# tbuckworth/train-procgen-pytorch

Hardware: AMD Instinct MI355X
Metric: env steps/sec (whole node), coinrun hard-500 IMPALA-CNN PPO (higher is better)
Workload: dtype bf16

## Files before the change

### train-procgen-pytorch_amd/csrc/common.h

```cpp
#pragma once
#include <hip/hip_runtime.h>
#include <stdint.h>
#include <stddef.h>

typedef float f32x4 __attribute__((ext_vector_type(4)));

#define MI_WAVE 64

#if defined(__HIPCC__)
typedef float mi_f32x2 __attribute__((ext_vector_type(2)));
typedef __bf16 mi_bf16x2 __attribute__((ext_vector_type(2)));
__device__ __forceinline__ unsigned mi_pk_bf16(float lo, float hi) {
    return __builtin_bit_cast(unsigned, __builtin_convertvector((mi_f32x2){lo, hi}, mi_bf16x2));
}

typedef short mi_s16x2 __attribute__((ext_vector_type(2)));
constexpr unsigned MI_KEY_MIN2 = 0x80008000u;
__device__ __forceinline__ unsigned mi_bf16x2_to_keys(unsigned w) {
    const mi_s16x2 v = __builtin_bit_cast(mi_s16x2, w), s = v >> (mi_s16x2){15, 15};
    return __builtin_bit_cast(unsigned, (mi_s16x2)((v ^ (s & (mi_s16x2){0x7fff, 0x7fff})) - s));
}
__device__ __forceinline__ unsigned mi_keys_to_bf16x2(unsigned kk) {
    mi_s16x2 k = __builtin_bit_cast(mi_s16x2, kk);
    const mi_s16x2 s = k >> (mi_s16x2){15, 15};
// ... 121 lines not shown
    int n, A;
    float inv_n_global;
    LossHP hp;
    int value_from_logits;
};
int  loss_blocks(int n);
void launch_loss_fwd(const LossArgs& a, hipStream_t st);
void launch_loss_finalize(const LossArgs& a, int nblk, int phase, const float* fs_ptr, float* log_slot, hipStream_t st);
void launch_logp_all(const float* hout, int n, int A, float* lp_out, float* value_out, hipStream_t st, int value_from_logits = 0);
void launch_loss_bwd(const LossArgs& a, hipStream_t st);
constexpr int MI_MAX_SEG = 16;
constexpr int FS_PARTS = 8;
struct SegTab { int n_seg; int start[MI_MAX_SEG + 1]; };
int  loss_blocks_seg(const SegTab& st);
void launch_loss_fwd_seg(const LossArgs& a, const SegTab& st, bool with_bwd, hipStream_t stream);
void launch_loss_finalize_seg(const LossArgs& a, const SegTab& st, int phase, float* stats_base, const double* fs_parts, int fs_d, float* fs_out,
                              float* log_base, hipStream_t stream);
void launch_loss_finalize_records(const LossArgs& a, int n_rec, float* stats_base, const float* fs_base, float* log_base, hipStream_t stream);
void launch_fs_metric_seg(const void* flat_pre, int bf16, const SegTab& st, int d, float* colmax_scratch, double* fs_parts, hipStream_t stream);
int  fs_groups_per_segment(int n_seg);
void launch_fs_grad(const void* x, int bf16, int n, int d, const float* part, int G, void* Gd, float fs_coef, float* colmax, int* arg, hipStream_t st);
void launch_fs_keys(const void* x, int bf16, int n, int d, const float* part, int G, const int32_t* gpos, float* colmax, int* arg,
                    long long* keys, long long* keys_local, hipStream_t st);
void launch_fs_apply_keys(void* Gd, int bf16, int d, const long long* keys, const long long* keys_local, const int* arg, float fs_coef, hipStream_t st);
void launch_fs_from_keys(const long long* keys, int d, float* fs_out, hipStream_t st);
int  fs_metric_groups();
void launch_fs_metric(const void* flat_pre, int bf16, int n, int d, float* colmax_scratch, float* fs_out, hipStream_t st);

void launch_gae(const float* rew, const float* done, const float* value, float* adv, float* ret, int T, int E,
                float gamma, float lmbda, int use_gae, hipStream_t st);
// ... 86 lines not shown
```

### train-procgen-pytorch_amd/csrc/engine.hip

```cpp
#include "engine_ctx.h"

thread_local std::string g_err;
thread_local hipStream_t tl_stream = nullptr;
thread_local float* tl_ws = nullptr;
thread_local size_t tl_ws_floats = 0;
const char* mi_last_error(void) { return g_err.c_str(); }

#define NCCLC(x)                                                                                         \
    do {                                                                                                 \
        ncclResult_t r_ = (x);                                                                           \
        if (r_ != ncclSuccess) return fail(-5, std::string(#x) + ": " + ncclGetErrorString(r_) + " @" + std::to_string(__LINE__)); \
    } while (0)

extern "C" int mi_comm_destroy(mi_ctx* c);
static void prof_harvest(mi_ctx* c);
static const char* kProfNames[PC_COUNT] = {
    "conv_fwd_3_16_64", "conv_fwd_16_16_32", "conv_fwd_16_32_32", "conv_fwd_32_32_16", "conv_fwd_32_32_8",
    "conv_dgrad_3_16_64(unused)", "conv_dgrad_16_16_32", "conv_dgrad_16_32_32", "conv_dgrad_32_32_16", "conv_dgrad_32_32_8",
    "conv_wgrad_3_16_64", "conv_wgrad_16_16_32", "conv_wgrad_16_32_32", "conv_wgrad_32_32_16", "conv_wgrad_32_32_8",
    "maxpool_fwd", "maxpool_bwd", "gemm", "slab_reduce",
    "resblock_fwd_(unused)", "resblock_fwd_16_16_32", "resblock_fwd_(unused)", "resblock_fwd_32_32_16", "resblock_fwd_32_32_8",
    "resblock_dgrad_(unused)", "resblock_dgrad_16_16_32", "resblock_dgrad_(unused)", "resblock_dgrad_32_32_16", "resblock_dgrad_32_32_8"};
struct GroupJob { int t; const void* frames; size_t bytes; bool pull; bool have_rd, last; const float* u; unsigned long long seed; unsigned ticket; };
struct GroupWorker {
// ... 137 lines not shown
            "impala out_dim (output_dim) must be a multiple of 64 in [64, 512]");
    int ndev = 0;
    if (hipGetDeviceCount(&ndev) != hipSuccess || ndev == 0) return fail(-3, "no HIP device: the MI355X library has no CPU fallback");
    HIPC(hipSetDevice(cfg->device));
    mi_ctx* c = new mi_ctx();
    c->cfg = *cfg;
    c->T = cfg->n_steps; c->E = cfg->n_envs; c->A = cfg->n_actions;
    c->H = (cfg->arch == MI_ARCH_IMPALA && cfg->out_dim == 0) ? 256 : cfg->out_dim;
    c->NB = cfg->max_batch < cfg->n_envs ? cfg->n_envs : cfg->max_batch;
    c->bf = (cfg->arch == MI_ARCH_IMPALA) && cfg->precision == 1;
    c->lse = cfg->value_from_logits;
    c->es = c->bf ? 2.0 : 4.0;
    if (cfg->stream) { c->stream = (hipStream_t)cfg->stream; c->own_stream = false; }
    else { HIPC(hipStreamCreateWithFlags(&c->stream, hipStreamNonBlocking)); c->own_stream = true; }
    HIPC(hipEventCreateWithFlags(&c->ev_side_fork, hipEventDisableTiming)); HIPC(hipEventCreateWithFlags(&c->ev_side_join, hipEventDisableTiming));
    c->side_stream = nullptr; c->side_on = true; c->side.armed = false;
    if (cfg->arch == MI_ARCH_IMPALA) build_impala_layout(c); else build_mlp_layout(c);
    if (cfg->arch == MI_ARCH_IMPALA && !impala_regions_ok(c)) { delete c; return fail(-1, "internal: parameter layout does not split at embedder.fc.weight"); }

    const int64_t P = c->n_params, T = c->T, E = c->E, NB = c->NB;
    HIPC(dalloc(&c->params, P)); HIPC(dalloc(&c->grads, P)); HIPC(dalloc(&c->adam_m, P)); HIPC(dalloc(&c->adam_v, P));
    HIPC(dalloc(&c->rew, T * E)); HIPC(dalloc(&c->done, T * E)); HIPC(dalloc(&c->logp, T * E));
    HIPC(dalloc(&c->adv, T * E)); HIPC(dalloc(&c->ret, T * E)); HIPC(dalloc(&c->value, (T + 1) * E));
    HIPC(dalloc(&c->act, T * E)); HIPC(dalloc(&c->adv_stats, 4));
    c->frames = nullptr; c->obsf = nullptr; c->stage_frames = nullptr; c->stage_obs = nullptr;
    if (cfg->arch == MI_ARCH_IMPALA) {
        c->obs_bytes_per_env = 64 * 64 * 3;
        HIPC(dalloc(&c->frames, (size_t)(T + 1) * E * c->obs_bytes_per_env));
        HIPC(dalloc(&c->stage_frames, (size_t)NB * c->obs_bytes_per_env));
        const int chan[4] = {3, 16, 32, 32};
        int hin = 64;
// ... 615 lines not shown
            conv_wgrad(c, L[0], c->blk[b - 1].P2, nullptr, 0, c->GC, n);
            conv_dgrad(c, L[0], c->GC, nullptr, nullptr, Gout, n);
        }
    }
    conv_wgrad_reduce_all(c, n);
    issue_grad_allreduce(c, 0, c->fc.w_off, true);
}

static void fork_stats_and_fc(mi_ctx* c, int n) {
    fc_refresh(c);
    const mi_ctx::SideJob& j = c->side;
    hipStream_t ss = side_stream(c);
    hipStreamWaitEvent(ss, c->ev_side_fork, 0);
    if (c->idx_ev_deferred >= 0) { hipEventRecord(c->idx_ev[c->idx_ev_deferred], ss); c->idx_ev_deferred = -1; }
    tl_stream = ss;
    launch_heads_bwd_reduce(c->gemm_ws, c->grads + c->wh_off, c->grads + c->bh_off, n, c->H, c->A + 1, ss);
    launch_fs_metric_seg(c->blk[2].P2, c->bf, j.st, 2048, c->fs_scratch, c->fs_parts, ss);
    launch_loss_finalize_seg(j.a, j.st, j.mode, j.ring, c->fs_parts, 2048, j.fsr, j.log, ss);
    launch_fc_tn(c->dfeat, (const unsigned short*)c->blk[2].P2, c->grads + c->fc.w_off, c->gemm_ws, (size_t)8 << 20, c->H, 2048, n, ss);
    launch_colsum_acc(c->dfeat, n, c->H, c->H, c->grads + c->fc.b_off, c->col_ws, ss);
    tl_stream = nullptr;
    hipEventRecord(c->ev_side_join, ss);
    c->side.armed = false;
}
static int fork_slab_sums(mi_ctx* c, bool fork_recorded) {
    hipStream_t ss = side_stream(c);
    int max_len = 0;
    for (int q = 0; q < c->slab_desc_n; ++q) max_len = std::max(max_len, c->h_slab_desc[q].slab_len);
    if (!fork_recorded) hipEventRecord(c->ev_side_fork, c->stream);
    hipStreamWaitEvent(ss, c->ev_side_fork, 0);
    launch_reduce_all_slabs(c->slabs, c->grads, c->d_slab_desc, c->slab_desc_n, max_len, ss);
// ... 76 lines not shown
        backward_conv_pool_bf16(c, b, n, Gout, Ga);
        std::swap(Gout, Ga);
    }
    const bool fork2_on_launch = backward_residual_pair(c, 0, n, Gout, Ga, Gb, fork2 ? c->ev_side_fork : nullptr);
    c->sal_src = Gout;
    int slabs_done = 0;
    if (fork2 && c->slab_desc_n >= 1) slabs_done = fork_slab_sums(c, fork2_on_launch);
    conv_wgrad(c, c->convs[0], nullptr, &src, 0, Gout, n, c->blk[0].PI);
    if (fork1 || slabs_done) hipStreamWaitEvent(c->stream, c->ev_side_join, 0);
    conv_wgrad_reduce_all(c, n, slabs_done);
    issue_grad_allreduce(c, 0, c->fc.w_off, true);
}

static void net_backward(mi_ctx* c, const InputSrc& src, int n) {
    const bool impala = c->cfg.arch == MI_ARCH_IMPALA;
    if (!c->bwd_from_dfeat) {
        const bool to_side = c->side.armed && !tl_stream;
        heads_backward(c, n, impala ? 1 : 0, c->H <= 256 && c->A + 1 <= 16 && !tl_ws, true, CUR(c), !to_side, to_side ? c->ev_side_fork : nullptr);
    }
    if (!impala) backward_mlp(c, n);
    else if (!c->bf) backward_impala_fp32(c, src, n);
    else backward_impala_bf16(c, src, n);
}

static int upload_u(mi_ctx* c, const float* u, hipStream_t st, int row0, int rows, const float** du) {
    *du = nullptr;
    if (u) { HIPC(hipMemcpyAsync(c->d_u + row0, u, (size_t)rows * 4, hipMemcpyHostToDevice, st)); *du = c->d_u + row0; }
    return 0;
}
static int read_back_staged(mi_ctx* c, const int32_t* d_act, const float* d_logp, const float* d_val, int64_t* act_out, float* logp_out, float* value_out, void* extra_out = nullptr, const void* d_extra = nullptr, size_t extra_bytes = 0) {
    const size_t E = c->E;
// ... 451 lines not shown
    a.value_from_logits = c->lse;
    a.hp = LossHP{hp->eps_clip, hp->value_coef, hp->entropy_coef, hp->x_entropy_coef, hp->entropy_multiplier, hp->fs_coef};
    return a;
}
static void loss_and_records(mi_ctx* c, const LossArgs& a, const SegTab& st, bool with_dY, int mode, float* ring, float* fsr, float* log) {
    const bool impala = c->cfg.arch == MI_ARCH_IMPALA;
    if (impala) launch_fs_metric_seg(c->blk[2].P2, c->bf, st, 2048, c->fs_scratch, c->fs_parts, c->stream);
    launch_loss_fwd_seg(a, st, with_dY, c->stream);
    launch_loss_finalize_seg(a, st, mode, ring, impala ? c->fs_parts : nullptr, 2048, fsr, log, c->stream);
}

static bool side_eligible(const mi_ctx* c, int n, bool batch_terms) {
    return c->side_on && c->cfg.arch == MI_ARCH_IMPALA && c->bf && n >= 1024 && !batch_terms && !c->ar_armed && !c->comm && !c->bwd_from_dfeat &&
           c->H <= 256 && c->A + 1 <= 16;
}
static int minibatch_impl(mi_ctx* c, const int64_t* idx, int32_t n, const int32_t* seg_n, int32_t n_seg, int32_t n_global, const mi_hparams* hp) {
    ARG(c && hp, "null"); JOIN(c); ARG(n >= 0 && n <= c->NB, "n_idx must be in [0, max_batch]"); ARG(n_global >= 1, "n_global");
    ARG(n == 0 || idx, "idx"); ARG(n_seg >= 1 && n_seg <= MI_MAX_SEG && seg_n, "1 .. 16 segments");
    ARG(c->log_count + n_seg <= c->log_cap, "loss log full: call mi_loss_log_read(reset=1)");
    ARG(c->pending_n < 0, "previous multirank minibatch not finished");
    { long long tot = 0; for (int k = 0; k < n_seg; ++k) { ARG(seg_n[k] >= 0, "negative segment"); tot += seg_n[k]; } ARG(tot == n, "segments do not add up to n_idx"); }
    const bool batch_terms = hp->x_entropy_coef != 0.f || hp->fs_coef != 0.f;
    ARG(hp->fs_coef == 0.f || c->multirank != 2, "fs_coef != 0 needs the column maxima over the GLOBAL minibatch before the backward pass: multirank mode 1");
    ARG(hp->fs_coef == 0.f || c->multirank == 0 || c->cfg.arch != MI_ARCH_IMPALA || c->gpos_n == n,
        "fs_coef != 0 on several ranks: call mi_minibatch_positions with this pass's global minibatch positions first");
    ARG(n_seg == 1 || (!batch_terms && c->multirank != 1), "several minibatches per call need x_entropy_coef == 0, fs_coef == 0 and multirank mode 0 or 2");
    const int64_t TE = (int64_t)c->T * c->E;
    for (int k = 0; k < n; ++k) ARG(idx[k] >= 0 && idx[k] < TE, "minibatch index out of range");
    if (n)
        if (int r = stage_indices(c, n, [&](int32_t* h) { for (int k = 0; k < n; ++k) h[k] = (int32_t)idx[k]; }, side_eligible(c, n, batch_terms) && c->multirank != 1)) return r;
    InputSrc src = minibatch_src(c);
    c->prof.phase = 1;
    c->prof.sample_now = (c->prof.mb_count++ % c->prof.period) == 0;
    c->rec_last = false;
    net_forward(c, src, n, {.train = true});
    const bool impala = c->cfg.arch == MI_ARCH_IMPALA;
    LossArgs a = loss_args(c, n, n_global, hp);
    if (c->multirank == 2)
        ARG(!batch_terms, "multirank mode 2 needs x_entropy_coef == 0 and fs_coef == 0 (use mode 1)");
    if (c->multirank != 1) {
        SegTab st{};
        st.n_seg = n_seg;
        for (int k = 0; k < n_seg; ++k) st.start[k + 1] = st.start[k] + seg_n[k];
        float* ring = c->stats_ring + (size_t)c->log_count * 32;
        float* fsr = c->fs_ring + c->log_count;
        a.stats = ring;
        const int mode = c->multirank == 2 ? 1 : 3;
        float* log = c->multirank == 2 ? nullptr : c->loss_log + (size_t)c->log_count * 8;
        if (side_eligible(c, n, batch_terms)) {
            launch_loss_fwd_seg(a, st, true, c->stream);
            c->side = mi_ctx::SideJob{true, a, st, mode, ring, fsr, log};
        } else
            loss_and_records(c, a, st, !batch_terms, mode, ring, fsr, log);
        c->ring_args = a;
        c->log_count += n_seg;
        if (batch_terms) launch_loss_bwd(a, c->stream);
        if (impala && hp->fs_coef != 0.f && n > 0) { c->fs_grad_coef = hp->fs_coef; c->fs_G = fs_groups_per_segment(n_seg); }
        net_backward(c, src, n);
        c->fs_grad_coef = 0.f;
        HIPC(hipGetLastError()); NETCHK(c);
        return 0;
    }
    if (impala) launch_fs_metric(c->blk[2].P2, c->bf, n, 2048, c->fs_scratch, c->fs_val, c->stream);
    c->fs_global_pending = impala && hp->fs_coef != 0.f;
    if (c->fs_global_pending) {
        if (n > 0) launch_fs_keys(c->blk[2].P2, c->bf, n, 2048, c->fs_scratch, fs_metric_groups(), c->d_gpos, c->fs_colmax, c->fs_arg, c->fs_keys, c->fs_keys_local, c->stream);
// ... 261 lines not shown
    return 0;
}

int mi_device_ptr(mi_ctx* c, int32_t which, void** ptr, int64_t* n) {
    ARG(c && ptr && n, "null"); JOIN(c);
    switch (which) {
        case MI_PTR_GRADS: *ptr = c->grads; *n = c->n_params; return 0;
        case MI_PTR_LOSS_STATS: *ptr = c->loss_stats; *n = 32; return 0;
        case MI_PTR_PARAMS: *ptr = c->params; *n = c->n_params; return 0;
        case MI_PTR_STATS_RING: *ptr = c->stats_ring; *n = (int64_t)c->log_cap * 32; return 0;
        case MI_PTR_FS_KEYS: ARG(c->fs_keys, "IMPALA contexts only"); *ptr = c->fs_keys; *n = 2048; return 0;
        default: return fail(-1, "unknown pointer id");
    }
}

int mi_debug_flags(mi_ctx* c, int32_t flags) { ARG(c, "null"); JOIN(c); c->rollout_tail = !(flags & 1); c->no_pull = (flags & 4) != 0; c->side_on = !(flags & 16); return 0; }
```

### train-procgen-pytorch_amd/csrc/engine_ctx.h

```cpp
#pragma once
#include "common.h"
#include "../../include/mi355ppo.h"
#include <rccl/rccl.h>
#include <math.h>
#include <stdio.h>
#include <string.h>
#include <string>
#include <unordered_map>
#include <vector>
#include <atomic>
#include <chrono>
#include <condition_variable>
#include <mutex>
#include <thread>

#pragma clang diagnostic ignored "-Wc++20-designator"
#define MI_INTERNAL __attribute__((visibility("hidden")))

MI_INTERNAL extern thread_local std::string g_err;
MI_INTERNAL extern thread_local hipStream_t tl_stream;
MI_INTERNAL extern thread_local float* tl_ws;
MI_INTERNAL extern thread_local size_t tl_ws_floats;
#define CUR(c) (tl_stream ? tl_stream : (c)->stream)
static inline int fail(int code, const std::string& msg) { g_err = msg; return code; }
// ... 84 lines not shown
    bool gru_on; float *gru_wih, *gru_whh, *gru_bih, *gru_bhh, *h_state, *h_masked, *gru_gi, *gru_gh, *d_done;
    float *gru_x, *gru_dg; bool sal_keep_x, bwd_from_dfeat;
    static constexpr int IDX_RING = 32;
    int32_t* h_idx_ring[IDX_RING]; hipEvent_t idx_ev[IDX_RING]; bool idx_used[IDX_RING]; int idx_next, idx_ev_deferred;
    float* h_f; int32_t* h_i; size_t h_f_floats;
    int multirank;
    LossArgs pending; int pending_n;
    static constexpr int MAX_GROUPS = 4;
    int n_groups; hipStream_t main_stream, gs[MAX_GROUPS]; hipEvent_t ev_fork[MAX_GROUPS], ev_join[MAX_GROUPS];
    bool g_forked[MAX_GROUPS], g_busy[MAX_GROUPS], g_last[MAX_GROUPS], g_dirty[MAX_GROUPS]; unsigned g_ticket[MAX_GROUPS]; bool groups_live;
    struct GroupWorker* gw[MAX_GROUPS];
    std::atomic<int64_t> copy_slot_ns{0}; double copy_rate_bytes_per_us;
    std::unordered_map<const void*, bool> pull_ok; bool no_pull;
    hipStream_t side_stream; hipEvent_t ev_side_fork, ev_side_join;
    bool side_on;
    struct SideJob { bool armed; LossArgs a; SegTab st; int mode; float* ring; float* fsr; float* log; } side;
    bool rollout_tail;
    float *fs_colmax, fs_grad_coef; int *fs_arg, fs_G;
    long long *fs_keys, *fs_keys_local; int32_t *d_gpos, *h_gpos; int gpos_n; bool fs_global_pending, fs_global_apply;
    ncclComm_t comm, comm_grad; int comm_world, comm_rank; hipStream_t comm_stream; hipEvent_t ev_ar_ready, ev_ar_done;
    bool ar_armed, ar_issued, ar_inflight; double* adv_all;
    std::string net_err; std::mutex net_err_mu;
    float *h_ring, *h_rec_stage; hipEvent_t ev_rec; bool g_rec_ok[MAX_GROUPS];
    bool gru_train, rec_last; float *gru_g, *gru_m, *gru_v; double* gru_sumsq;
    float *rec_x, *rec_gi, *rec_sv, *rec_dgi, *rec_dgh, *rec_hm, *rec_mask, *rec_h0;
};

static inline char* obs_ring(mi_ctx* c) { return c->frames ? (char*)c->frames : (char*)c->obsf; }

MI_INTERNAL std::string net_err_take(mi_ctx* c);
MI_INTERNAL void net_err_set(mi_ctx* c, const std::string& m);
// ... 19 lines not shown
```

### train-procgen-pytorch_amd/csrc/engine_ops.hip

```cpp
#include "engine_ctx.h"

static int shape_of(int cin, int cout, int hw, ConvShape* s) {
    for (int k = 0; k < CS_COUNT; ++k) {
        int a, b, h; conv_shape_dims((ConvShape)k, &a, &b, &h);
        if (a == cin && b == cout && h == hw) { *s = (ConvShape)k; return 0; }
    }
    return fail(-1, "unsupported conv shape");
}

std::vector<uint16_t> host_to_bf16(const float* x, size_t n) {
    std::vector<uint16_t> o(n);
    for (size_t k = 0; k < n; ++k) { uint32_t u; memcpy(&u, x + k, 4); o[k] = (uint16_t)((u + 0x7FFFu + ((u >> 16) & 1u)) >> 16); }
    return o;
}
static void host_from_bf16(const uint16_t* h, float* x, size_t n) {
    for (size_t k = 0; k < n; ++k) { const uint32_t u = ((uint32_t)h[k]) << 16; memcpy(x + k, &u, 4); }
}
struct OpMem {
    static constexpr size_t GUARD = 64 * 1024;
    static constexpr int CANARY = 0xA5;
    struct Band { std::string name; unsigned char* p; size_t bytes; bool rezero; };
    const char* hook; hipStream_t st;
    std::vector<void*> owned;
    std::vector<Band> bands;
// ... 369 lines not shown
    if (graph) hipGraphDestroy(graph);
    c->prof.on = prof_on;
    HIPC(hipGetLastError()); NETCHK(c);
    return 0;
}

int mi_debug_read(mi_ctx* c, int32_t which, int32_t n, float* out) {
    ARG(c && out, "null"); JOIN(c); ARG(n >= 1 && n <= c->NB, "n must be in [1, max_batch]");
    if (which == 100 || which == 101 || which == 102) {
        ARG(which == 100 || c->rec_last, "which = 101 / 102: only after mi_minibatch_rec");
        const float* srcp = which == 102 ? c->dfeat : (which == 100 && c->rec_last) ? c->rec_x : c->feat;
        HIPC(hipMemcpyAsync(out, srcp, (size_t)n * c->H * 4, hipMemcpyDeviceToHost, c->stream));
        HIPC(hipStreamSynchronize(c->stream));
        return 0;
    }
    ARG(c->cfg.arch == MI_ARCH_IMPALA && which >= 0 && which < 24 && (which & 7) <= 5, "which");
    const Block& k = c->blk[which >> 3];
    const size_t pe = (size_t)n * (k.hin / 2) * (k.hin / 2) * k.cout;
    HIPC(hipStreamSynchronize(c->stream));
    if ((which & 7) == 5) {
        std::vector<uint8_t> h(pe);
        HIPC(hipMemcpy(h.data(), k.PI, pe, hipMemcpyDeviceToHost));
        for (size_t i = 0; i < pe; ++i) out[i] = (float)h[i];
        return 0;
    }
    const float* src[5] = {k.P0, k.A1, k.P1, k.A2, k.P2};
    return download_act(c, src[which & 7], out, pe);
}

int mi_op_maxpool(mi_ctx* c, int32_t mode, int32_t n, int32_t hw, int32_t ch, const float* in, const float* dout, float* out) {
// ... 63 lines not shown
```

### train-procgen-pytorch_amd/csrc/misc.hip

```cpp
#include "common.h"
#include <hip/hip_ext.h>
#include <math.h>
#include <stdlib.h>

static thread_local const char* tl_launch_err = nullptr;
void mi_launch_fail(const char* msg) { if (!tl_launch_err) tl_launch_err = msg; }
const char* mi_launch_failed_take() { const char* m = tl_launch_err; tl_launch_err = nullptr; return m; }

#define MFMA16(a, b, c) __builtin_amdgcn_mfma_f32_16x16x4f32((a), (b), (c), 0, 0, 0)

template <typename T>
__device__ __forceinline__ T wave_sum(T v) {
#pragma unroll
    for (int o = 32; o > 0; o >>= 1) v += __shfl_down(v, o, 64);
    return v;
}
__device__ __forceinline__ float wave_max(float v) {
#pragma unroll
    for (int o = 32; o > 0; o >>= 1) v = fmaxf(v, __shfl_down(v, o, 64));
    return v;
}
template <typename T>
__device__ __forceinline__ T block_sum256(T v, T* sbuf) {
    v = wave_sum(v);
// ... 380 lines not shown
            for (int q = 0; q < 8; ++q) v[q] = dY[(long long)(m + q * groups) * ld + n];
#pragma unroll
            for (int q = 0; q < 8; ++q) s += v[q];
        }
        for (; m < M; m += groups) s += dY[(long long)m * ld + n];
        part[(long long)rg * N + n] = s;
    }
}
void launch_colsum_acc(const float* dY, int M, int N, int ld, float* db, float* col_ws, hipStream_t st) {
    if (M <= 0) return;
    const int gy = (M >= 4096 && N <= 1024) ? 64 : 16;
    hipLaunchKernelGGL(colsum_partial_kernel, dim3((N + 63) / 64, gy), dim3(256), 0, st, dY, M, N, ld, col_ws);
    launch_reduce_slabs(col_ws, gy * 4, N, db, N, nullptr, 0, st);
}

__global__ __launch_bounds__(256) void heads_fwd_kernel(const float* __restrict__ feat, const float* __restrict__ Wh, const float* __restrict__ bh,
                                                        float* __restrict__ hout, int n, int O) {
    __shared__ __attribute__((aligned(16))) float s_f[16 * 260];
    __shared__ __attribute__((aligned(16))) float s_w[16 * 260];
    const int tid = threadIdx.x, e0 = blockIdx.x * 16, el = tid >> 4, o = tid & 15;
    f32x4 rf[4], rw[4];
#pragma unroll
    for (int j = 0; j < 4; ++j) {
        const int k = tid + j * 256, r = k >> 6, kk = (k & 63) * 4;
        const int rr = e0 + r < n ? e0 + r : n - 1;
        rf[j] = *(const f32x4*)(feat + (long long)rr * 256 + kk);
        rw[j] = *(const f32x4*)(Wh + (long long)(r < O ? r : O - 1) * 256 + kk);
    }
#pragma unroll
    for (int j = 0; j < 4; ++j) { const int k = tid + j * 256; *(f32x4*)(s_f + (k >> 6) * 260 + (k & 63) * 4) = rf[j]; *(f32x4*)(s_w + (k >> 6) * 260 + (k & 63) * 4) = rw[j]; }
    __syncthreads();
    const float* w = s_w + o * 260;
    const float* f = s_f + el * 260;
    float acc = 0.f;
#pragma unroll 8
    for (int k = 0; k < 256; k += 4) {
        const f32x4 fv = *(const f32x4*)(f + k), ww = *(const f32x4*)(w + k);
        acc += fv.x * ww.x + fv.y * ww.y + fv.z * ww.z + fv.w * ww.w;
    }
    if (o < O && e0 + el < n) hout[(long long)(e0 + el) * O + o] = acc + bh[o];
}
void launch_heads_fwd(const float* feat, const float* Wh, const float* bh, float* hout, int n, int O, hipStream_t st) {
    if (n <= 0) return;
    hipLaunchKernelGGL(heads_fwd_kernel, dim3((n + 15) / 16), dim3(256), 0, st, feat, Wh, bh, hout, n, O);
}

typedef const __attribute__((address_space(4))) float* hb_const_f32p;
__global__ __launch_bounds__(256) void heads_bwd_kernel(const float* __restrict__ dY, const float* __restrict__ feat, const float* __restrict__ Wh,
                                                        int relu_mask, float* __restrict__ dfeat, float* __restrict__ slab, int n, int H, int O) {
    const int k = threadIdx.x;
    const int chunk = (n + gridDim.x - 1) / gridDim.x, r0 = blockIdx.x * chunk, r1 = min(n, r0 + chunk);
    float w[16], gw[16], gb = 0.f;
#pragma unroll
    for (int o = 0; o < 16; ++o) { w[o] = (o < O && k < H) ? Wh[(long long)o * H + k] : 0.f; gw[o] = 0.f; }
// ... 26 lines not shown
        for (int o = 0; o < 16; ++o) if (o < O) { const float v = dy[o]; acc = fmaf(v, w[o], acc); gw[o] = fmaf(v, f, gw[o]); }
        if (k < H) dfeat[(long long)s * H + k] = (relu_mask && !(f > 0.f)) ? 0.f : acc;
        if (k < O) gb += dY[(long long)s * O + k];
    }
    float* sl = slab + (long long)blockIdx.x * (O * H + O);
    if (k < H) {
#pragma unroll
        for (int o = 0; o < 16; ++o) if (o < O) sl[(long long)o * H + k] = gw[o];
    }
    if (k < O) sl[(long long)O * H + k] = gb;
}
static int heads_bwd_grid(int n) { const int g = (n + 15) / 16; return g > 512 ? 512 : g; }
void launch_heads_bwd_reduce(const float* ws, float* gW, float* gb, int n, int H, int O, hipStream_t st) {
    if (n <= 0) return;
    launch_reduce_slabs(ws, heads_bwd_grid(n), O * H + O, gW, O * H, gb, O, st);
}
void launch_heads_bwd(const float* dY, const float* feat, const float* Wh, int relu_mask, float* dfeat, float* gW, float* gb, float* ws,
                      int n, int H, int O, hipStream_t st, bool with_reduce, hipEvent_t done_ev) {
    if (n <= 0) return;
    if (done_ev) hipExtLaunchKernelGGL(heads_bwd_kernel, dim3(heads_bwd_grid(n)), dim3(256), 0, st, nullptr, done_ev, 0, dY, feat, Wh, relu_mask, dfeat, ws, n, H, O);
    else
    hipLaunchKernelGGL(heads_bwd_kernel, dim3(heads_bwd_grid(n)), dim3(256), 0, st, dY, feat, Wh, relu_mask, dfeat, ws, n, H, O);
    if (with_reduce) launch_heads_bwd_reduce(ws, gW, gb, n, H, O, st);
}

__global__ void gather_rows_kernel(const float* src, const int32_t* idx, long long base, float* dst, int n, int d) {
    const long long e = (long long)blockIdx.x * blockDim.x + threadIdx.x;
    if (e >= (long long)n * d) return;
    const int s = e / d, c = e % d;
    const long long row = idx ? (long long)idx[s] : base + s;
// ... 29 lines not shown
    float s = 0.f;
#pragma unroll
    for (int a = 0; a < MAXA; ++a) if (a < A) s += expf(z[a] - mx);
    const float lse = mx + logf(s);
    float s2 = 0.f;
#pragma unroll
    for (int a = 0; a < MAXA; ++a) if (a < A) { lp[a] = z[a] - lse; const float e1 = expf(lp[a]); s2 += e1; if (LSE) q1[a] = e1; }
    if (LSE) lse_out = lse;
    const float lse2 = logf(s2);
    float s3 = 0.f;
#pragma unroll
    for (int a = 0; a < MAXA; ++a) if (a < A) { lp[a] -= lse2; p[a] = expf(lp[a]); s3 += p[a]; }
#pragma unroll
    for (int a = 0; a < MAXA; ++a) if (a < A) p[a] /= s3;
}
template <bool LSE>
__device__ __forceinline__ void sample_terms(const LossArgs& a, int s, SampleTerms& t) {
    const float* h = a.hout + (long long)s * (a.A + 1);
    float z[MAXA];
#pragma unroll
    for (int k = 0; k < MAXA; ++k) z[k] = (k < a.A) ? h[k] : 0.f;
    float lse = 0.f;
    log_softmax_twice_t<LSE>(z, a.A, t.lp, t.p, lse, t.q1);
    const int gi = a.idx[s];
    t.act = a.act[gi];
    t.adv = a.adv[gi]; t.ret = a.ret[gi]; t.oldv = a.old_value[gi];
    t.v = LSE ? lse : h[a.A];
    float H = 0.f, lp_act = 0.f;
#pragma unroll
    for (int k = 0; k < MAXA; ++k) if (k < a.A) { H -= t.p[k] * t.lp[k]; lp_act = (k == t.act) ? t.lp[k] : lp_act; }
    t.H = H;
    t.ratio = expf(lp_act - a.old_logp[gi]);
    t.surr1 = t.ratio * t.adv;
    t.surr2 = fminf(fmaxf(t.ratio, 1.f - a.hp.eps_clip), 1.f + a.hp.eps_clip) * t.adv;
    t.vclip = t.oldv + fminf(fmaxf(t.v - t.oldv, -a.hp.eps_clip), a.hp.eps_clip);
    t.vs1 = (t.v - t.ret) * (t.v - t.ret);
    t.vs2 = (t.vclip - t.ret) * (t.vclip - t.ret);
}

constexpr int LOSS_BLK = 64;
int loss_blocks(int n) { return (n + LOSS_BLK - 1) / LOSS_BLK; }

template <bool LSE>
__device__ __forceinline__ void loss_bwd_sample(const LossArgs& a, int s, const SampleTerms& t) {
    const float ib = a.inv_n_global;
    const float dvl = t.v - t.oldv;
    const float inr = (dvl >= -a.hp.eps_clip && dvl <= a.hp.eps_clip) ? 1.f : 0.f;
    float gv;
    if (t.vs1 > t.vs2) gv = 2.f * (t.v - t.ret);
    else if (t.vs2 > t.vs1) gv = 2.f * (t.vclip - t.ret) * inr;
    else gv = (t.v - t.ret) + (t.vclip - t.ret) * inr;
    const float gvc = a.hp.value_coef * 0.5f * ib * gv;
    const float g_lp = -ib * ((t.surr1 <= t.surr2) ? t.adv : 0.f) * t.ratio;
    const float cH = (-a.hp.entropy_coef * a.hp.entropy_mult + a.hp.x_entropy_coef) * ib;
    float plq = 0.f;
    float lq[MAXA];
    const bool xe = a.hp.x_entropy_coef != 0.f;
    if (xe) {
#pragma unroll
        for (int k = 0; k < MAXA; ++k) if (k < a.A) { lq[k] = logf(a.stats[8 + k]); plq += t.p[k] * lq[k]; }
    }
    float* d = a.dY + (long long)s * (a.A + 1);
#pragma unroll
    for (int k = 0; k < MAXA; ++k) if (k < a.A) {
        float gk = g_lp * ((k == t.act ? 1.f : 0.f) - t.p[k]);
        gk += cH * (-t.p[k] * (t.lp[k] + t.H));
        if (xe) gk += a.hp.x_entropy_coef * ib * t.p[k] * (lq[k] - plq);
        if (LSE) gk += gvc * t.q1[k];
        d[k] = gk;
    }
    d[a.A] = LSE ? 0.f : gvc;
}
template <bool LSE>
__global__ __launch_bounds__(LOSS_BLK) void loss_bwd_kernel(LossArgs a) {
    const int s = blockIdx.x * LOSS_BLK + threadIdx.x;
    if (s >= a.n) return;
    SampleTerms t;
    sample_terms<LSE>(a, s, t);
    loss_bwd_sample<LSE>(a, s, t);
}
template <bool BWD, bool LSE>
__device__ __forceinline__ void loss_fwd_block(const LossArgs& a, int s, int s_end, int row) {
    constexpr int NW = LOSS_BLK / 64;
    __shared__ float sw[NW][8 + MAXA];
    SampleTerms t;
    float pi = 0.f, vm = 0.f, H = 0.f;
// ... 43 lines not shown
    loss_fwd_block<BWD, LSE>(a, st.start[k] + (blockIdx.x - first) * LOSS_BLK + threadIdx.x, st.start[k + 1], blockIdx.x);
}
int loss_blocks_seg(const SegTab& st) {
    int nb = 0;
    for (int k = 0; k < st.n_seg; ++k) nb += (st.start[k + 1] - st.start[k] + LOSS_BLK - 1) / LOSS_BLK;
    return nb;
}
void launch_loss_fwd_seg(const LossArgs& a, const SegTab& st, bool with_bwd, hipStream_t stream) {
    const int nb = loss_blocks_seg(st);
    if (nb <= 0) return;
    if (a.value_from_logits) {
        if (with_bwd) hipLaunchKernelGGL((loss_fwd_seg_kernel<true, true>), dim3(nb), dim3(LOSS_BLK), 0, stream, a, st);
        else hipLaunchKernelGGL((loss_fwd_seg_kernel<false, true>), dim3(nb), dim3(LOSS_BLK), 0, stream, a, st);
    } else if (with_bwd) hipLaunchKernelGGL((loss_fwd_seg_kernel<true, false>), dim3(nb), dim3(LOSS_BLK), 0, stream, a, st);
    else hipLaunchKernelGGL((loss_fwd_seg_kernel<false, false>), dim3(nb), dim3(LOSS_BLK), 0, stream, a, st);
}
void launch_loss_fwd(const LossArgs& a, hipStream_t st) {
    if (a.n <= 0) return;
    if (a.value_from_logits) hipLaunchKernelGGL(loss_fwd_kernel<true>, dim3(loss_blocks(a.n)), dim3(LOSS_BLK), 0, st, a);
    else hipLaunchKernelGGL(loss_fwd_kernel<false>, dim3(loss_blocks(a.n)), dim3(LOSS_BLK), 0, st, a);
}

__device__ __forceinline__ void loss_finalize_body(const LossArgs& a, int nblk, int phase, const float* fs_ptr, float* log_slot) {
    const int k = threadIdx.x;
    if (phase & 1) {
        __shared__ float sp[8][32];
        const int c = k & 31, g = k >> 5, G = blockDim.x >> 5;
        const bool col = c < 3 || (c >= 8 && c < 8 + a.A);
        float s = 0.f;
        if (col && g < 8) for (int b = g; b < nblk; b += G) s += a.partial[(long long)b * (8 + a.A) + c];
// ... 889 lines not shown
```

### train-procgen-pytorch_amd/mi355/engine.py

```python
import ctypes as C
import os

import numpy as np

_HERE = os.path.dirname(os.path.abspath(__file__))
_LIB = None

ARCH_IMPALA, ARCH_MLP = 0, 1
F_REW, F_DONE, F_VALUE, F_LOGP, F_ADV, F_RET, F_ACT = range(7)
PTR_GRADS, PTR_LOSS_STATS, PTR_PARAMS, PTR_STATS_RING, PTR_FS_KEYS = 0, 1, 2, 3, 4
LOSS_FIELDS = ("pi_loss", "value_loss", "entropy", "x_ent", "total", "fs", "marg", "_pad")


class EngineError(RuntimeError):
    pass


class _Config(C.Structure):
    _fields_ = [("arch", C.c_int32), ("n_steps", C.c_int32), ("n_envs", C.c_int32), ("n_actions", C.c_int32),
                ("obs_dim", C.c_int32), ("mlp_depth", C.c_int32), ("mlp_width", C.c_int32), ("out_dim", C.c_int32),
                ("max_batch", C.c_int32), ("device", C.c_int32), ("precision", C.c_int32), ("value_from_logits", C.c_int32),
                ("reserved", C.c_int32 * 4),
                ("stream", C.c_void_p)]

# ... 496 lines not shown

    def op_gemm(self, A, B, transpose_a=False, transpose_b=False):
        A, B = _f32(A), _f32(B)
        M, K = (A.shape[1], A.shape[0]) if transpose_a else A.shape
        N = B.shape[0] if transpose_b else B.shape[1]
        sam, sak = (1, A.shape[1]) if transpose_a else (A.shape[1], 1)
        sbk, sbn = (1, B.shape[1]) if transpose_b else (B.shape[1], 1)
        out = np.empty((M, N), np.float32)
        self._chk(self.lib.mi_op_gemm(self._ctx, C.c_int32(M), C.c_int32(N), C.c_int32(K), _fp(A), C.c_int64(sam),
                                      C.c_int64(sak), _fp(B), C.c_int64(sbk), C.c_int64(sbn), _fp(out)))
        return out

    def debug_read(self, which, n):
        if which in (100, 101, 102):
            out = np.empty((n, self.H), np.float32)
        else:
            b = which >> 3
            hw, ch = (32, 16, 8)[b], (16, 32, 32)[b]
            out = np.empty((n, hw, hw, ch), np.float32)
        self._chk(self.lib.mi_debug_read(self._ctx, C.c_int32(which), C.c_int32(n), _fp(out)))
        return out

    def minibatch_positions(self, gpos):
        g = np.ascontiguousarray(gpos, dtype=np.int32)
        self._chk(self.lib.mi_minibatch_positions(self._ctx, g.ctypes.data_as(C.c_void_p), C.c_int32(g.size)))

    def debug_philox(self, ctr_key6):
        a = np.ascontiguousarray(ctr_key6, dtype=np.uint32).reshape(-1, 6)
        out, u = np.empty((a.shape[0], 4), np.uint32), np.empty(a.shape[0], np.float32)
        self._chk(self.lib.mi_debug_philox(self._ctx, _fp(a), C.c_int32(a.shape[0]), _fp(out), _fp(u)))
# ... 24 lines not shown
```

Before: 609,400.

## Fuse policy/value heads forward, PPO loss and heads backward into one kernel

Adds a single kernel per loss block that computes the linear heads' outputs, the PPO loss terms and partials, dY, dfeat and per-block weight-gradient slabs, replacing separate heads-forward, loss-forward/backward and heads-backward launches on the side-stream path. The goal is to cut kernel launches and the round trips of hout and dY through global memory. The side job then reduces the fused slabs with a new reduce variant. This uses 1024-thread blocks with large dynamic LDS, adds more slabs to reduce, and is gated by a debug flag and by eligibility conditions.

```diff
diff --git a/train-procgen-pytorch_amd/csrc/common.h b/train-procgen-pytorch_amd/csrc/common.h
--- a/train-procgen-pytorch_amd/csrc/common.h
+++ b/train-procgen-pytorch_amd/csrc/common.h
@@ -159,6 +159,10 @@
 struct SegTab { int n_seg; int start[MI_MAX_SEG + 1]; };
 int  loss_blocks_seg(const SegTab& st);
 void launch_loss_fwd_seg(const LossArgs& a, const SegTab& st, bool with_bwd, hipStream_t stream);
+int  heads_loss_bwd_slabs(const SegTab& st);
+void launch_heads_loss_bwd(const float* feat, const float* Wh, const float* bh, float* hout, const LossArgs& a, const SegTab& st, float* dfeat, float* slab,
+                           hipStream_t stream, hipEvent_t done_ev);
+void launch_heads_bwd_reduce_n(const float* ws, int nslab, float* gW, float* gb, int H, int O, hipStream_t st);
 void launch_loss_finalize_seg(const LossArgs& a, const SegTab& st, int phase, float* stats_base, const double* fs_parts, int fs_d, float* fs_out,
                               float* log_base, hipStream_t stream);
 void launch_loss_finalize_records(const LossArgs& a, int n_rec, float* stats_base, const float* fs_base, float* log_base, hipStream_t stream);
diff --git a/train-procgen-pytorch_amd/csrc/engine.hip b/train-procgen-pytorch_amd/csrc/engine.hip
--- a/train-procgen-pytorch_amd/csrc/engine.hip
+++ b/train-procgen-pytorch_amd/csrc/engine.hip
@@ -175,7 +175,7 @@
     if (cfg->stream) { c->stream = (hipStream_t)cfg->stream; c->own_stream = false; }
     else { HIPC(hipStreamCreateWithFlags(&c->stream, hipStreamNonBlocking)); c->own_stream = true; }
     HIPC(hipEventCreateWithFlags(&c->ev_side_fork, hipEventDisableTiming)); HIPC(hipEventCreateWithFlags(&c->ev_side_join, hipEventDisableTiming));
-    c->side_stream = nullptr; c->side_on = true; c->side.armed = false;
+    c->side_stream = nullptr; c->side_on = true; c->side.armed = false; c->chain_fused = true; c->heads_done = false;
     if (cfg->arch == MI_ARCH_IMPALA) build_impala_layout(c); else build_mlp_layout(c);
     if (cfg->arch == MI_ARCH_IMPALA && !impala_regions_ok(c)) { delete c; return fail(-1, "internal: parameter layout does not split at embedder.fc.weight"); }
 
@@ -821,7 +821,8 @@
     hipStreamWaitEvent(ss, c->ev_side_fork, 0);
     if (c->idx_ev_deferred >= 0) { hipEventRecord(c->idx_ev[c->idx_ev_deferred], ss); c->idx_ev_deferred = -1; }
     tl_stream = ss;
-    launch_heads_bwd_reduce(c->gemm_ws, c->grads + c->wh_off, c->grads + c->bh_off, n, c->H, c->A + 1, ss);
+    if (j.heads_slabs > 0) launch_heads_bwd_reduce_n(c->gemm_ws, j.heads_slabs, c->grads + c->wh_off, c->grads + c->bh_off, c->H, c->A + 1, ss);
+    else launch_heads_bwd_reduce(c->gemm_ws, c->grads + c->wh_off, c->grads + c->bh_off, n, c->H, c->A + 1, ss);
     launch_fs_metric_seg(c->blk[2].P2, c->bf, j.st, 2048, c->fs_scratch, c->fs_parts, ss);
     launch_loss_finalize_seg(j.a, j.st, j.mode, j.ring, c->fs_parts, 2048, j.fsr, j.log, ss);
     launch_fc_tn(c->dfeat, (const unsigned short*)c->blk[2].P2, c->grads + c->fc.w_off, c->gemm_ws, (size_t)8 << 20, c->H, 2048, n, ss);
@@ -928,7 +929,9 @@
 
 static void net_backward(mi_ctx* c, const InputSrc& src, int n) {
     const bool impala = c->cfg.arch == MI_ARCH_IMPALA;
-    if (!c->bwd_from_dfeat) {
+    const bool heads_done = c->heads_done;
+    c->heads_done = false;
+    if (!c->bwd_from_dfeat && !heads_done) {
         const bool to_side = c->side.armed && !tl_stream;
         heads_backward(c, n, impala ? 1 : 0, c->H <= 256 && c->A + 1 <= 16 && !tl_ws, true, CUR(c), !to_side, to_side ? c->ev_side_fork : nullptr);
     }
@@ -1410,6 +1413,12 @@
     return c->side_on && c->cfg.arch == MI_ARCH_IMPALA && c->bf && n >= 1024 && !batch_terms && !c->ar_armed && !c->comm && !c->bwd_from_dfeat &&
            c->H <= 256 && c->A + 1 <= 16;
 }
+static SegTab seg_table(const int32_t* seg_n, int n_seg) {
+    SegTab st{};
+    st.n_seg = n_seg;
+    for (int k = 0; k < n_seg; ++k) st.start[k + 1] = st.start[k] + seg_n[k];
+    return st;
+}
 static int minibatch_impl(mi_ctx* c, const int64_t* idx, int32_t n, const int32_t* seg_n, int32_t n_seg, int32_t n_global, const mi_hparams* hp) {
     ARG(c && hp, "null"); JOIN(c); ARG(n >= 0 && n <= c->NB, "n_idx must be in [0, max_batch]"); ARG(n_global >= 1, "n_global");
     ARG(n == 0 || idx, "idx"); ARG(n_seg >= 1 && n_seg <= MI_MAX_SEG && seg_n, "1 .. 16 segments");
@@ -1429,23 +1438,29 @@
     c->prof.phase = 1;
     c->prof.sample_now = (c->prof.mb_count++ % c->prof.period) == 0;
     c->rec_last = false;
-    net_forward(c, src, n, {.train = true});
+    const SegTab seg = seg_table(seg_n, n_seg);
+    const bool fuse = c->chain_fused && c->multirank != 1 && side_eligible(c, n, batch_terms) && c->H == 256 && !tl_stream &&
+                      (size_t)heads_loss_bwd_slabs(seg) * (size_t)((c->A + 1) * 257) <= c->gemm_ws_floats;
+    net_forward(c, src, n, {.heads = !fuse, .train = true});
     const bool impala = c->cfg.arch == MI_ARCH_IMPALA;
     LossArgs a = loss_args(c, n, n_global, hp);
     if (c->multirank == 2)
         ARG(!batch_terms, "multirank mode 2 needs x_entropy_coef == 0 and fs_coef == 0 (use mode 1)");
     if (c->multirank != 1) {
-        SegTab st{};
-        st.n_seg = n_seg;
-        for (int k = 0; k < n_seg; ++k) st.start[k + 1] = st.start[k] + seg_n[k];
+        const SegTab& st = seg;
         float* ring = c->stats_ring + (size_t)c->log_count * 32;
         float* fsr = c->fs_ring + c->log_count;
         a.stats = ring;
         const int mode = c->multirank == 2 ? 1 : 3;
         float* log = c->multirank == 2 ? nullptr : c->loss_log + (size_t)c->log_count * 8;
         if (side_eligible(c, n, batch_terms)) {
-            launch_loss_fwd_seg(a, st, true, c->stream);
-            c->side = mi_ctx::SideJob{true, a, st, mode, ring, fsr, log};
+            if (fuse) {
+                ProfScope ps(c, PC_GEMM, n, 4.0 * (2.0 * n * (c->A + 1) + 2.0 * n * c->H + (double)c->H * (c->A + 1)), 6.0 * n * c->H * (c->A + 1));
+                launch_heads_loss_bwd(c->feat, c->params + c->wh_off, c->params + c->bh_off, c->hout, a, st, c->dfeat, c->gemm_ws, c->stream, c->ev_side_fork);
+                c->heads_done = true;
+            } else
+                launch_loss_fwd_seg(a, st, true, c->stream);
+            c->side = mi_ctx::SideJob{true, a, st, mode, ring, fsr, log, fuse ? heads_loss_bwd_slabs(st) : 0};
         } else
             loss_and_records(c, a, st, !batch_terms, mode, ring, fsr, log);
         c->ring_args = a;
@@ -1737,4 +1752,4 @@
     }
 }
 
-int mi_debug_flags(mi_ctx* c, int32_t flags) { ARG(c, "null"); JOIN(c); c->rollout_tail = !(flags & 1); c->no_pull = (flags & 4) != 0; c->side_on = !(flags & 16); return 0; }
+int mi_debug_flags(mi_ctx* c, int32_t flags) { ARG(c, "null"); JOIN(c); c->rollout_tail = !(flags & 1); c->no_pull = (flags & 4) != 0; c->side_on = !(flags & 16); c->chain_fused = !(flags & 32); return 0; }
diff --git a/train-procgen-pytorch_amd/csrc/engine_ctx.h b/train-procgen-pytorch_amd/csrc/engine_ctx.h
--- a/train-procgen-pytorch_amd/csrc/engine_ctx.h
+++ b/train-procgen-pytorch_amd/csrc/engine_ctx.h
@@ -122,7 +122,9 @@
     std::unordered_map<const void*, bool> pull_ok; bool no_pull;
     hipStream_t side_stream; hipEvent_t ev_side_fork, ev_side_join;
     bool side_on;
-    struct SideJob { bool armed; LossArgs a; SegTab st; int mode; float* ring; float* fsr; float* log; } side;
+    struct SideJob { bool armed; LossArgs a; SegTab st; int mode; float* ring; float* fsr; float* log; int heads_slabs;  } side;
+    bool chain_fused;
+    bool heads_done;
     bool rollout_tail;
     float *fs_colmax, fs_grad_coef; int *fs_arg, fs_G;
     long long *fs_keys, *fs_keys_local; int32_t *d_gpos, *h_gpos; int gpos_n; bool fs_global_pending, fs_global_apply;
diff --git a/train-procgen-pytorch_amd/csrc/engine_ops.hip b/train-procgen-pytorch_amd/csrc/engine_ops.hip
--- a/train-procgen-pytorch_amd/csrc/engine_ops.hip
+++ b/train-procgen-pytorch_amd/csrc/engine_ops.hip
@@ -407,6 +407,13 @@
         HIPC(hipStreamSynchronize(c->stream));
         return 0;
     }
+    if (which >= 103 && which <= 105) {
+        const float* srcp = which == 103 ? c->hout : which == 104 ? c->dY : c->dfeat;
+        const size_t row = which == 105 ? (size_t)c->H : (size_t)c->A + 1;
+        HIPC(hipMemcpyAsync(out, srcp, (size_t)n * row * 4, hipMemcpyDeviceToHost, c->stream));
+        HIPC(hipStreamSynchronize(c->stream));
+        return 0;
+    }
     ARG(c->cfg.arch == MI_ARCH_IMPALA && which >= 0 && which < 24 && (which & 7) <= 5, "which");
     const Block& k = c->blk[which >> 3];
     const size_t pe = (size_t)n * (k.hin / 2) * (k.hin / 2) * k.cout;
diff --git a/train-procgen-pytorch_amd/csrc/misc.hip b/train-procgen-pytorch_amd/csrc/misc.hip
--- a/train-procgen-pytorch_amd/csrc/misc.hip
+++ b/train-procgen-pytorch_amd/csrc/misc.hip
@@ -1,6 +1,7 @@
 #include "common.h"
 #include <hip/hip_ext.h>
 #include <math.h>
+#include <mutex>
 #include <stdlib.h>
 
 static thread_local const char* tl_launch_err = nullptr;
@@ -418,6 +419,15 @@
     launch_reduce_slabs(col_ws, gy * 4, N, db, N, nullptr, 0, st);
 }
 
+__device__ __forceinline__ float heads_dot256(const float* f, const float* w) {
+    float acc = 0.f;
+#pragma unroll 8
+    for (int k = 0; k < 256; k += 4) {
+        const f32x4 fv = *(const f32x4*)(f + k), ww = *(const f32x4*)(w + k);
+        acc += fv.x * ww.x + fv.y * ww.y + fv.z * ww.z + fv.w * ww.w;
+    }
+    return acc;
+}
 __global__ __launch_bounds__(256) void heads_fwd_kernel(const float* __restrict__ feat, const float* __restrict__ Wh, const float* __restrict__ bh,
                                                         float* __restrict__ hout, int n, int O) {
     __shared__ __attribute__((aligned(16))) float s_f[16 * 260];
@@ -434,14 +444,7 @@
 #pragma unroll
     for (int j = 0; j < 4; ++j) { const int k = tid + j * 256; *(f32x4*)(s_f + (k >> 6) * 260 + (k & 63) * 4) = rf[j]; *(f32x4*)(s_w + (k >> 6) * 260 + (k & 63) * 4) = rw[j]; }
     __syncthreads();
-    const float* w = s_w + o * 260;
-    const float* f = s_f + el * 260;
-    float acc = 0.f;
-#pragma unroll 8
-    for (int k = 0; k < 256; k += 4) {
-        const f32x4 fv = *(const f32x4*)(f + k), ww = *(const f32x4*)(w + k);
-        acc += fv.x * ww.x + fv.y * ww.y + fv.z * ww.z + fv.w * ww.w;
-    }
+    const float acc = heads_dot256(s_f + el * 260, s_w + o * 260);
     if (o < O && e0 + el < n) hout[(long long)(e0 + el) * O + o] = acc + bh[o];
 }
 void launch_heads_fwd(const float* feat, const float* Wh, const float* bh, float* hout, int n, int O, hipStream_t st) {
@@ -498,6 +501,9 @@
 void launch_heads_bwd_reduce(const float* ws, float* gW, float* gb, int n, int H, int O, hipStream_t st) {
     if (n <= 0) return;
     launch_reduce_slabs(ws, heads_bwd_grid(n), O * H + O, gW, O * H, gb, O, st);
+}
+void launch_heads_bwd_reduce_n(const float* ws, int nslab, float* gW, float* gb, int H, int O, hipStream_t st) {
+    launch_reduce_slabs(ws, nslab, O * H + O, gW, O * H, gb, O, st);
 }
 void launch_heads_bwd(const float* dY, const float* feat, const float* Wh, int relu_mask, float* dfeat, float* gW, float* gb, float* ws,
                       int n, int H, int O, hipStream_t st, bool with_reduce, hipEvent_t done_ev) {
@@ -557,35 +563,42 @@
 #pragma unroll
     for (int a = 0; a < MAXA; ++a) if (a < A) p[a] /= s3;
 }
+struct SampleIn { int act; float adv, ret, oldv, old_logp; };
+__device__ __forceinline__ SampleIn sample_gather(const LossArgs& a, int s) {
+    const int gi = a.idx[s];
+    return SampleIn{a.act[gi], a.adv[gi], a.ret[gi], a.old_value[gi], a.old_logp[gi]};
+}
 template <bool LSE>
-__device__ __forceinline__ void sample_terms(const LossArgs& a, int s, SampleTerms& t) {
-    const float* h = a.hout + (long long)s * (a.A + 1);
+__device__ __forceinline__ void sample_terms_from(const LossArgs& a, const float* h, const SampleIn& in, SampleTerms& t) {
     float z[MAXA];
 #pragma unroll
     for (int k = 0; k < MAXA; ++k) z[k] = (k < a.A) ? h[k] : 0.f;
     float lse = 0.f;
     log_softmax_twice_t<LSE>(z, a.A, t.lp, t.p, lse, t.q1);
-    const int gi = a.idx[s];
-    t.act = a.act[gi];
-    t.adv = a.adv[gi]; t.ret = a.ret[gi]; t.oldv = a.old_value[gi];
+    t.act = in.act;
+    t.adv = in.adv; t.ret = in.ret; t.oldv = in.oldv;
     t.v = LSE ? lse : h[a.A];
     float H = 0.f, lp_act = 0.f;
 #pragma unroll
     for (int k = 0; k < MAXA; ++k) if (k < a.A) { H -= t.p[k] * t.lp[k]; lp_act = (k == t.act) ? t.lp[k] : lp_act; }
     t.H = H;
-    t.ratio = expf(lp_act - a.old_logp[gi]);
+    t.ratio = expf(lp_act - in.old_logp);
     t.surr1 = t.ratio * t.adv;
     t.surr2 = fminf(fmaxf(t.ratio, 1.f - a.hp.eps_clip), 1.f + a.hp.eps_clip) * t.adv;
     t.vclip = t.oldv + fminf(fmaxf(t.v - t.oldv, -a.hp.eps_clip), a.hp.eps_clip);
     t.vs1 = (t.v - t.ret) * (t.v - t.ret);
     t.vs2 = (t.vclip - t.ret) * (t.vclip - t.ret);
 }
+template <bool LSE>
+__device__ __forceinline__ void sample_terms(const LossArgs& a, int s, SampleTerms& t) {
+    sample_terms_from<LSE>(a, a.hout + (long long)s * (a.A + 1), sample_gather(a, s), t);
+}
 
 constexpr int LOSS_BLK = 64;
 int loss_blocks(int n) { return (n + LOSS_BLK - 1) / LOSS_BLK; }
 
 template <bool LSE>
-__device__ __forceinline__ void loss_bwd_sample(const LossArgs& a, int s, const SampleTerms& t) {
+__device__ __forceinline__ void loss_bwd_sample_to(const LossArgs& a, float* d, const SampleTerms& t) {
     const float ib = a.inv_n_global;
     const float dvl = t.v - t.oldv;
     const float inr = (dvl >= -a.hp.eps_clip && dvl <= a.hp.eps_clip) ? 1.f : 0.f;
@@ -603,7 +616,6 @@
 #pragma unroll
         for (int k = 0; k < MAXA; ++k) if (k < a.A) { lq[k] = logf(a.stats[8 + k]); plq += t.p[k] * lq[k]; }
     }
-    float* d = a.dY + (long long)s * (a.A + 1);
 #pragma unroll
     for (int k = 0; k < MAXA; ++k) if (k < a.A) {
         float gk = g_lp * ((k == t.act ? 1.f : 0.f) - t.p[k]);
@@ -613,6 +625,10 @@
         d[k] = gk;
     }
     d[a.A] = LSE ? 0.f : gvc;
+}
+template <bool LSE>
+__device__ __forceinline__ void loss_bwd_sample(const LossArgs& a, int s, const SampleTerms& t) {
+    loss_bwd_sample_to<LSE>(a, a.dY + (long long)s * (a.A + 1), t);
 }
 template <bool LSE>
 __global__ __launch_bounds__(LOSS_BLK) void loss_bwd_kernel(LossArgs a) {
@@ -686,6 +702,111 @@
         else hipLaunchKernelGGL((loss_fwd_seg_kernel<false, true>), dim3(nb), dim3(LOSS_BLK), 0, stream, a, st);
     } else if (with_bwd) hipLaunchKernelGGL((loss_fwd_seg_kernel<true, false>), dim3(nb), dim3(LOSS_BLK), 0, stream, a, st);
     else hipLaunchKernelGGL((loss_fwd_seg_kernel<false, false>), dim3(nb), dim3(LOSS_BLK), 0, stream, a, st);
+}
+
+constexpr int HL_ROWS = LOSS_BLK, HL_LDS_FLOATS = HL_ROWS * 260 + 16 * 260 + HL_ROWS * 17 + HL_ROWS * 16 + 32;
+template <bool LSE>
+__global__ __launch_bounds__(1024) void heads_loss_bwd_kernel(const float* __restrict__ feat, const float* __restrict__ Wh, const float* __restrict__ bh,
+                                                              float* __restrict__ hout, LossArgs a, SegTab st, float* __restrict__ dfeat, float* __restrict__ slab) {
+    extern __shared__ __attribute__((aligned(16))) float hl_smem[];
+    float* s_f = hl_smem;
+    float* s_w = s_f + HL_ROWS * 260;
+    float* s_h = s_w + 16 * 260;
+    float* s_d = s_h + HL_ROWS * 17;
+    float* s_p = s_d + HL_ROWS * 16;
+    const int tid = threadIdx.x, O = a.A + 1;
+    int seg, first;
+    seg_of_block(st, blockIdx.x, seg, first);
+    const int row0 = st.start[seg] + (blockIdx.x - first) * HL_ROWS, s_end = st.start[seg + 1];
+    SampleIn in{};
+    if (tid < HL_ROWS && row0 + tid < s_end) in = sample_gather(a, row0 + tid);
+    {
+        f32x4 rf[4];
+#pragma unroll
+        for (int j = 0; j < 4; ++j) {
+            const int k = tid + j * 1024, r = k >> 6, kk = (k & 63) * 4;
+            const int rr = row0 + r < s_end ? row0 + r : s_end - 1;
+            rf[j] = *(const f32x4*)(feat + (long long)rr * 256 + kk);
+        }
+        const int wr = tid >> 6, wk = (tid & 63) * 4;
+        const f32x4 rw = *(const f32x4*)(Wh + (long long)(wr < O ? wr : O - 1) * 256 + wk);
+#pragma unroll
+        for (int j = 0; j < 4; ++j) { const int k = tid + j * 1024; *(f32x4*)(s_f + (k >> 6) * 260 + (k & 63) * 4) = rf[j]; }
+        *(f32x4*)(s_w + wr * 260 + wk) = rw;
+    }
+    __syncthreads();
+    {
+        const int el = tid >> 4, o = tid & 15;
+        const float acc = heads_dot256(s_f + el * 260, s_w + o * 260);
+        if (o < O) {
+            const float hv = acc + bh[o];
+            s_h[el * 17 + o] = hv;
+            if (row0 + el < s_end) hout[(long long)(row0 + el) * O + o] = hv;
+        }
+    }
+    __syncthreads();
+    if (tid < 64) {
+        SampleTerms t;
+        float pi = 0.f, vm = 0.f, H = 0.f;
+        float pa[MAXA];
+#pragma unroll
+        for (int k = 0; k < MAXA; ++k) pa[k] = 0.f;
+        if (row0 + tid < s_end) {
+            sample_terms_from<LSE>(a, s_h + tid * 17, in, t);
+            pi = fminf(t.surr1, t.surr2);
+            vm = fmaxf(t.vs1, t.vs2);
+            H = t.H;
+#pragma unroll
+            for (int k = 0; k < MAXA; ++k) if (k < a.A) pa[k] = t.p[k];
+            loss_bwd_sample_to<LSE>(a, s_d + tid * 16, t);
+        }
+        float r = wave_sum(pi); if (tid == 0) s_p[0] = r;
+        r = wave_sum(vm);       if (tid == 0) s_p[1] = r;
+        r = wave_sum(H);        if (tid == 0) s_p[2] = r;
+#pragma unroll
+        for (int k = 0; k < MAXA; ++k) if (k < a.A) { r = wave_sum(pa[k]); if (tid == 0) s_p[8 + k] = r; }
+    }
+    __syncthreads();
+    if (tid < 3 || (tid >= 8 && tid < 8 + a.A)) a.partial[(long long)blockIdx.x * (8 + a.A) + tid] = s_p[tid];
+    {
+        const int r = tid >> 4, o = tid & 15;
+        if (o < O && row0 + r < s_end) a.dY[(long long)(row0 + r) * O + o] = s_d[r * 16 + o];
+    }
+    {
+        const int g = tid >> 8, k = tid & 255;
+        float w[16], gw[16], gb = 0.f;
+#pragma unroll
+        for (int o = 0; o < 16; ++o) { w[o] = o < O ? s_w[o * 260 + k] : 0.f; gw[o] = 0.f; }
+        const int r1 = min(g * 16 + 16, s_end - row0);
+#pragma unroll 4
+        for (int r = g * 16; r < r1; ++r) {
+            const float f = s_f[r * 260 + k];
+            const float* dy = s_d + r * 16;
+            float acc = 0.f;
+#pragma unroll
+            for (int o = 0; o < 16; ++o) if (o < O) { const float v = dy[o]; acc = fmaf(v, w[o], acc); gw[o] = fmaf(v, f, gw[o]); }
+            dfeat[(long long)(row0 + r) * 256 + k] = !(f > 0.f) ? 0.f : acc;
+            if (k < O) gb += dy[k];
+        }
+        float* sl = slab + ((long long)blockIdx.x * 4 + g) * (O * 256 + O);
+#pragma unroll
+        for (int o = 0; o < 16; ++o) if (o < O) sl[(long long)o * 256 + k] = gw[o];
+        if (k < O) sl[(long long)O * 256 + k] = gb;
+    }
+}
+int heads_loss_bwd_slabs(const SegTab& st) { return 4 * loss_blocks_seg(st); }
+void launch_heads_loss_bwd(const float* feat, const float* Wh, const float* bh, float* hout, const LossArgs& a, const SegTab& st, float* dfeat, float* slab,
+                           hipStream_t stream, hipEvent_t done_ev) {
+    const int nb = loss_blocks_seg(st);
+    if (nb <= 0) return;
+    constexpr size_t LDS = HL_LDS_FLOATS * sizeof(float);
+    static std::once_flag attr;
+    std::call_once(attr, [] {
+        hipFuncSetAttribute((const void*)heads_loss_bwd_kernel<false>, hipFuncAttributeMaxDynamicSharedMemorySize, (int)LDS);
+        hipFuncSetAttribute((const void*)heads_loss_bwd_kernel<true>, hipFuncAttributeMaxDynamicSharedMemorySize, (int)LDS);
+    });
+    if (a.value_from_logits) hipExtLaunchKernelGGL(heads_loss_bwd_kernel<true>, dim3(nb), dim3(1024), LDS, stream, nullptr, done_ev, 0, feat, Wh, bh, hout, a, st, dfeat, slab);
+    else hipExtLaunchKernelGGL(heads_loss_bwd_kernel<false>, dim3(nb), dim3(1024), LDS, stream, nullptr, done_ev, 0, feat, Wh, bh, hout, a, st, dfeat, slab);
 }
 void launch_loss_fwd(const LossArgs& a, hipStream_t st) {
     if (a.n <= 0) return;
diff --git a/train-procgen-pytorch_amd/mi355/engine.py b/train-procgen-pytorch_amd/mi355/engine.py
--- a/train-procgen-pytorch_amd/mi355/engine.py
+++ b/train-procgen-pytorch_amd/mi355/engine.py
@@ -534,6 +534,8 @@
     def debug_read(self, which, n):
         if which in (100, 101, 102):
             out = np.empty((n, self.H), np.float32)
+        elif which in (103, 104, 105):
+            out = np.empty((n, self.H if which == 105 else self.A + 1), np.float32)
         else:
             b = which >> 3
             hw, ch = (32, 16, 8)[b], (16, 32, 32)[b]
```

After: 611,200 (median of 2 runs). No clear change (+0.3%).
